# qc-tum/TNC

Measured on NVIDIA H100. Metric: pairwise contractions/sec (effective ZGEMM TFLOP/s in zgemm_tflops), higher is better.
Workload: dtype f64

## Files before the change

### tnc_b200/csrc/crt.cu

```cuda
#include "internal.h"
#include "sm90.h"
#include <cuda.h>
#include <algorithm>
#include <cmath>
#include <cstdio>
#include <cstdlib>

namespace tncb {

constexpr int CRT_MAX_MOD = 20;
static const int kModuli[CRT_MAX_MOD] = {256, 253, 251, 249, 247, 245, 241, 239, 233, 229,
                                         227, 223, 211, 199, 197, 193, 191, 181, 179, 173};
constexpr int CRT_BT = 128;
constexpr int CRT_BKB = 128;
template <bool KARA> struct CrtRing {
  static constexpr int STAGES = KARA ? 3 : 2;
};
constexpr int CRT_STG_ROW = 2 * CRT_BT + 16;
constexpr int CRT_STG_BYTES = 64 * CRT_STG_ROW;
constexpr int CRT_KCHUNK_MAX = 32768;
constexpr int CRT_G = 34;

struct CrtTables {
  int nmod;
  int a_bits_a, a_bits_b;
  int mod[CRT_MAX_MOD];
  int magic[CRT_MAX_MOD];
  double inv_mod[CRT_MAX_MOD];
  double rho1[CRT_MAX_MOD];
  double rho2[CRT_MAX_MOD];
  double p_scaled;
};

double crt_log2_product(int n) {
  double s = 0;
  for (int i = 0; i < n; i++) s += std::log2((double)kModuli[i]);
  return s;
}

void crt_choose(long long K, int want_bits, int nmod_force, int* nmod, int* bits_a, int* bits_b) {
  const double lk = std::log2((double)std::max<long long>(K, 1));
  auto needed = [&](int bits) {
    int q = 2;
    while (q < CRT_MAX_MOD && crt_log2_product(q) - 1e-9 < 2.0 * bits + lk + 3.0) q++;
    return q;
  };
  int n = nmod_force > 0 ? std::min(nmod_force, needed(53)) : needed(want_bits);
  n = std::max(2, std::min(n, CRT_MAX_MOD));
  int tot = (int)std::floor(crt_log2_product(n) - lk - 3.0 - 1e-9);
  tot = std::max(tot, 2);
  int a = std::min(want_bits, tot / 2), b = std::min(want_bits, tot - a);
  *nmod = n; *bits_a = a; *bits_b = b;
// ... 202 lines not shown
struct CrtGemmArgs {
  int8_t* R;
  int Np, Mp;
  int tiles_n, tiles_m, tile_m;
  int nmod, nkc, kb_per_chunk, num_kb;
  int total_items;
  int group;
  int negmod[CRT_MAX_MOD];
  int magic[CRT_MAX_MOD];
};

struct CrtItem { int mod_i, prod, kc, n0, m0; };
template <bool KARA>
__device__ __forceinline__ CrtItem crt_decode(const CrtGemmArgs& p, int item) {
  const int tiles = p.tiles_n * p.tiles_m;
  const int mk = item / tiles, t = item - mk * tiles;
  CrtItem it;
  const int mp = mk / p.nkc;
  it.kc = mk - mp * p.nkc;
  it.mod_i = KARA ? mp / 3 : mp; it.prod = KARA ? mp - it.mod_i * 3 : 0;
  const int per_band = p.group * p.tiles_m;
  const int band = t / per_band, first = band * p.group;
  const int gsize = min(p.group, p.tiles_n - first);
  const int r = t - band * per_band;
  it.n0 = (first + r % gsize) * CRT_BT;
  it.m0 = (r / gsize) * p.tile_m;
  return it;
}

template <bool KARA>
__global__ void __launch_bounds__(WG_THREADS, 1)
crt_gemm_kernel(const __grid_constant__ CUtensorMap mapB, const __grid_constant__ CUtensorMap mapA,
                const __grid_constant__ CrtGemmArgs p) {
  constexpr int STAGES = CrtRing<KARA>::STAGES;
  extern __shared__ __align__(1024) uint8_t crt_smem_raw[];
  uint8_t* smem = reinterpret_cast<uint8_t*>((reinterpret_cast<uintptr_t>(crt_smem_raw) + 1023) & ~(uintptr_t)1023);
  __shared__ uint64_t full_bar[STAGES], empty_bar[STAGES];
  const int wg = threadIdx.x >> 7, tid = threadIdx.x & 127;

  if (threadIdx.x == 0) {
    for (int s = 0; s < STAGES; s++) { wg_mbar_init(&full_bar[s], 1); wg_mbar_init(&empty_bar[s], 2); }
    asm volatile("fence.mbarrier_init.release.cluster;" ::: "memory");
  }
  __syncthreads();

  if (wg == 0) {
    wg_setmaxnreg_producer();
    if (tid != 0) return;
    int it = 0;
    for (int item = blockIdx.x; item < p.total_items; item += gridDim.x) {
      const CrtItem w = crt_decode<KARA>(p, item);
      const int kb0 = w.kc * p.kb_per_chunk, kb1 = min(p.num_kb, kb0 + p.kb_per_chunk);
      const int rowB = (KARA ? w.mod_i * 3 + w.prod : w.mod_i * 2) * p.Np + w.n0;
      const int rowA = (KARA ? w.mod_i * 3 + w.prod : w.mod_i * 3) * p.Mp + w.m0;
      for (int kb = kb0; kb < kb1; kb++, it++) {
        uint8_t* st = wg_produce_begin<STAGES, KARA>(smem, full_bar, empty_bar, it);
        uint64_t* bar = &full_bar[it % STAGES];
        const int kx = kb * CRT_BKB;
        uint8_t* a = st + WgStage<KARA>::A;
        wg_tma_2d(&mapB, bar, st, kx, rowB);
        if (KARA) {
          wg_tma_2d(&mapA, bar, a, kx, rowA);
          wg_tma_2d(&mapA, bar, a + WG_TILE, kx, rowA + WG_ROWS);
        } else {
          wg_tma_2d(&mapB, bar, st + WgStage<KARA>::B1, kx, rowB + p.Np);
          wg_tma_2d(&mapA, bar, a, kx, rowA);
          wg_tma_2d(&mapA, bar, a + WG_TILE, kx, rowA + p.Mp);
          wg_tma_2d(&mapA, bar, a + 2 * WG_TILE, kx, rowA + 2 * p.Mp);
        }
      }
    }
  } else {
    wg_setmaxnreg_consumer();
    const int c = wg - 1, wq = tid >> 5, lane = tid & 31;
    WgRing<STAGES, KARA> ring{smem, full_bar, empty_bar};
    uint8_t* stg = smem + STAGES * WgStage<KARA>::BYTES + c * CRT_STG_BYTES;
    uint32_t acc[128];
#pragma unroll
    for (int i = 0; i < 128; i++) acc[i] = 0u;
    for (int item = blockIdx.x; item < p.total_items; item += gridDim.x) {
      const CrtItem w = crt_decode<KARA>(p, item);
      const int kb0 = w.kc * p.kb_per_chunk, kb1 = min(p.num_kb, kb0 + p.kb_per_chunk);
      bool first = true;
      for (int kb = kb0; kb < kb1; kb++) ring.mma_stage(acc, c, first, tid == 0);
      ring.drain(tid == 0);
      const int negm = p.negmod[w.mod_i], magic = p.magic[w.mod_i];
      wg_bar_sync(1 + c);
#pragma unroll
      for (int j = 0; j < 32; j++) {
#pragma unroll
        for (int h = 0; h < 2; h++) {
          uint32_t b = 0;
#pragma unroll
          for (int e = 0; e < 2; e++) {
            const int a = (int)acc[4 * j + 2 * h + e];
            int t = __mulhi(a, magic) * negm + a;
            if (t > 127) t += negm;
            b |= ((uint32_t)t & 0xffu) << (8 * e);
          }
          const int r = wq * 16 + (lane >> 2) + 8 * h, col = 8 * j + 2 * (lane & 3);
          *reinterpret_cast<uint16_t*>(stg + r * CRT_STG_ROW + col) = (uint16_t)(b ^ 0x8080u);
        }
      }
      wg_bar_sync(1 + c);
      const long long nrow0 = (long long)w.n0 + c * 64;
#pragma unroll
      for (int i = 0; i < 8; i++) {
        const int q = i * 128 + tid, row = q >> 4, c16 = q & 15;
        int8_t* dst = KARA ? p.R + ((long long)((w.mod_i * p.nkc + w.kc) * 3 + w.prod) * p.Np + nrow0 + row) * p.Mp + w.m0 + c16 * 16
                           : p.R + ((long long)((w.mod_i * p.nkc + w.kc) * 2 + (c16 >> 3)) * p.Np + nrow0 + row) * p.Mp + w.m0 + (c16 & 7) * 16;
        *reinterpret_cast<uint4*>(dst) = *reinterpret_cast<const uint4*>(stg + row * CRT_STG_ROW + c16 * 16);
      }
    }
  }
}

struct CrtReconArgs {
  const int8_t* R;
  double2* C;
  const unsigned long long* max_n;
  const unsigned long long* max_m;
  long long rows, cols, ldc;
  long long Np, Mp;
  int nkc;
};

template <bool ONE_CHUNK, bool KARA>
__global__ void __launch_bounds__(256, 4)
crt_reconstruct_kernel(const __grid_constant__ CrtReconArgs a, const __grid_constant__ CrtTables T) {
  const long long cols4 = a.Mp >> 2;
  const long long idx = (long long)blockIdx.x * blockDim.x + threadIdx.x;
  const long long n = idx / cols4, m4 = (idx - n * cols4) * 4;
  if (n >= a.rows || m4 >= a.cols) return;
  double s1r[4], s2r[4], s1i[4], s2i[4];
#pragma unroll
  for (int j = 0; j < 4; j++) { s1r[j] = s2r[j] = s1i[j] = s2i[j] = 0.0; }
  const long long plane = a.Np * a.Mp;
  const int8_t* base = a.R + n * a.Mp + m4;
  const double bias = 4503599627370496.0 + (KARA ? 256.0 : 128.0) * (double)a.nkc;
  const double bias_i = 4503599627370496.0 + (KARA ? 384.0 : 128.0) * (double)a.nkc;
#pragma unroll 8
  for (int i = 0; i < T.nmod; i++) {
    uint32_t ur[4], ui[4];
    if (KARA) {
// ... 40 lines not shown
  double2* dst = a.C + n * a.ldc + m4;
  const double RMAGIC = 6755399441055744.0;
#pragma unroll
  for (int j = 0; j < 4; j++) {
    if (m4 + j >= a.cols) break;
    const int em = crt_exp_from_bits(a.max_m[m4 + j]);
    double2 out;
    if (en == kExpNonFinite || em == kExpNonFinite) {
      out = make_double2(__longlong_as_double(0x7ff8000000000000LL), __longlong_as_double(0x7ff8000000000000LL));
    } else {
      const double qr = ((s1r[j] + s2r[j]) + RMAGIC) - RMAGIC;
      const double qi = ((s1i[j] + s2i[j]) + RMAGIC) - RMAGIC;
      const double fr = (s1r[j] - qr) + s2r[j], fi = (s1i[j] - qi) + s2i[j];
      out = make_double2(scalbn(fr * T.p_scaled, en + em), scalbn(fi * T.p_scaled, en + em));
    }
    dst[j] = out;
  }
}

typedef CUresult (*EncodeTiledFn)(CUtensorMap*, CUtensorMapDataType, cuuint32_t, void*, const cuuint64_t*, const cuuint64_t*,
                                  const cuuint32_t*, const cuuint32_t*, CUtensorMapInterleave, CUtensorMapSwizzle,
                                  CUtensorMapL2promotion, CUtensorMapFloatOOBfill);
static EncodeTiledFn get_encode() {
  static EncodeTiledFn fn = nullptr;
  static bool tried = false;
  if (!tried) {
    tried = true;
    cudaDriverEntryPointQueryResult q;
    void* p = nullptr;
    if (cudaGetDriverEntryPoint("cuTensorMapEncodeTiled", &p, cudaEnableDefault, &q) == cudaSuccess) fn = (EncodeTiledFn)p;
  }
  return fn;
}
int wg_make_map(CUtensorMap* m, void* ptr, uint64_t rows, uint64_t kbytes) {
  EncodeTiledFn enc = get_encode();
  if (!enc) return fail(TNCB_ERR_CUDA, "cuTensorMapEncodeTiled is not available");
  cuuint64_t dims[2] = {kbytes, rows};
  cuuint64_t strides[1] = {kbytes};
  cuuint32_t box[2] = {(cuuint32_t)WG_BKB, (cuuint32_t)WG_ROWS};
  cuuint32_t estr[2] = {1, 1};
  CUresult r = enc(m, CU_TENSOR_MAP_DATA_TYPE_UINT8, 2, ptr, dims, strides, box, estr, CU_TENSOR_MAP_INTERLEAVE_NONE,
                   CU_TENSOR_MAP_SWIZZLE_128B, CU_TENSOR_MAP_L2_PROMOTION_L2_256B, CU_TENSOR_MAP_FLOAT_OOB_FILL_NONE);
  if (r != CUDA_SUCCESS) return fail(TNCB_ERR_CUDA, "cuTensorMapEncodeTiled failed: " + std::to_string((int)r));
  return TNCB_OK;
}

static inline long long round_up_ll(long long x, long long a) { return (x + a - 1) / a * a; }


int launch_k1_crt(tncb_ctx* ctx, const PairPlan& P, const double2* A, const double2* B, double2* C,
                  const long long* offAm, const long long* offBn, const long long* offAk, const long long* offBk) {
  int nmod, bits_a, bits_b;
  const int want = ctx->crt_tol > 0.0 ? crt_bits_for_tolerance(P.K, ctx->crt_tol) : ctx->crt_bits;
  crt_choose(P.K, want, ctx->crt_nmod_force, &nmod, &bits_a, &bits_b);
  CrtTables T;
  crt_make_tables(nmod, bits_a, bits_b, T);
  cudaStream_t st = ctx->stream;
  const long long Kp = round_up_ll(P.K, CRT_BKB);
  const int num_kb = (int)(Kp / CRT_BKB);
  const int ctas_max = std::max(1, ctx->sm_count);
  const bool kara = ctx->crt_products == 3 || (ctx->crt_products == 0 && Kp >= ctx->crt_kara_min_k);
  const int TM = kara ? 2 * CRT_BT : CRT_BT;
  const int NPB = kara ? 3 : 2, NPR = kara ? 3 : 2;
  const long long tiles_total = round_up_ll(P.N, CRT_BT) / CRT_BT * (round_up_ll(P.M, TM) / TM);
  int nkc = (int)((Kp + CRT_KCHUNK_MAX - 1) / CRT_KCHUNK_MAX);
  {
    const long long items = tiles_total * nmod * (kara ? 3 : 1);
    const long long want = ctas_max;
    if (items * nkc < want) nkc = (int)std::min<long long>((want + items - 1) / items, std::max(1, num_kb / 8));
    nkc = std::max(1, std::min(nkc, 32));
  }
  int kb_per_chunk = (num_kb + nkc - 1) / nkc;
  nkc = (num_kb + kb_per_chunk - 1) / kb_per_chunk;
  if ((long long)kb_per_chunk * CRT_BKB > CRT_KCHUNK_MAX) return fail(TNCB_ERR_UNSUPPORTED, "K too long for the int8 engine");

  const size_t budget = ctx->crt_ws_bytes;
  long long pn = round_up_ll(P.N, CRT_BT), pm = round_up_ll(P.M, TM);
  auto ws_bytes = [&](long long n_, long long m_) {
    return (size_t)nmod * (size_t)Kp * (size_t)(NPB * n_ + 3 * m_) + (size_t)nmod * nkc * NPR * (size_t)n_ * (size_t)m_;
  };
  while (ws_bytes(pn, pm) > budget && (pm > TM || pn > CRT_BT)) {
    if (pm >= pn && pm > TM) pm = round_up_ll(pm / 2, TM);
    else if (pn > CRT_BT) pn = round_up_ll(pn / 2, CRT_BT);
    else pm = round_up_ll(pm / 2, TM);
  }
  const size_t bytesB = (size_t)nmod * NPB * pn * Kp, bytesA = (size_t)nmod * 3 * pm * Kp;
  const size_t bytesR = (size_t)nmod * nkc * NPR * pn * pm;
  const size_t bytesE = (size_t)(pn + pm) * sizeof(unsigned long long);
  void *pb = nullptr, *pa = nullptr, *pr = nullptr, *pe = nullptr;
  int rc;
  if ((rc = ctx->arena.alloc(bytesB, &pb))) return rc;
  if ((rc = ctx->arena.alloc(bytesA, &pa))) { ctx->arena.free(pb, bytesB); return rc; }
  if ((rc = ctx->arena.alloc(bytesR, &pr))) { ctx->arena.free(pb, bytesB); ctx->arena.free(pa, bytesA); return rc; }
  if ((rc = ctx->arena.alloc(bytesE, &pe))) { ctx->arena.free(pb, bytesB); ctx->arena.free(pa, bytesA); ctx->arena.free(pr, bytesR); return rc; }
  auto cleanup = [&]() { ctx->arena.free(pb, bytesB); ctx->arena.free(pa, bytesA); ctx->arena.free(pr, bytesR); ctx->arena.free(pe, bytesE); };
  unsigned long long* max_n = (unsigned long long*)pe;
  unsigned long long* max_m = max_n + pn;

  static bool attr_done_dev[64] = {false};
  bool& attr_done = attr_done_dev[ctx->device & 63];
  const int smem_gemm4 = CrtRing<false>::STAGES * WgStage<false>::BYTES + 2 * CRT_STG_BYTES + 1024;
  const int smem_gemm3 = CrtRing<true>::STAGES * WgStage<true>::BYTES + 2 * CRT_STG_BYTES + 1024;
  const int smem_res = RES_ROWS * RES_RS * (int)sizeof(double2);
  if (!attr_done) {
    cudaError_t e = cudaFuncSetAttribute(crt_gemm_kernel<false>, cudaFuncAttributeMaxDynamicSharedMemorySize, smem_gemm4);
    if (e == cudaSuccess) e = cudaFuncSetAttribute(crt_gemm_kernel<true>, cudaFuncAttributeMaxDynamicSharedMemorySize, smem_gemm3);
    if (e == cudaSuccess) e = cudaFuncSetAttribute(crt_residue_kernel<2, false>, cudaFuncAttributeMaxDynamicSharedMemorySize, smem_res);
    if (e == cudaSuccess) e = cudaFuncSetAttribute(crt_residue_kernel<3, false>, cudaFuncAttributeMaxDynamicSharedMemorySize, smem_res);
    if (e == cudaSuccess) e = cudaFuncSetAttribute(crt_residue_kernel<2, true>, cudaFuncAttributeMaxDynamicSharedMemorySize, smem_res);
    if (e == cudaSuccess) e = cudaFuncSetAttribute(crt_residue_kernel<3, true>, cudaFuncAttributeMaxDynamicSharedMemorySize, smem_res);
    if (e != cudaSuccess) { cleanup(); return fail(TNCB_ERR_CUDA, cudaGetErrorString(e)); }
    attr_done = true;
  }
  auto lane_split = [](const LegList& kl, bool k_is_b, const LegList& fl) {
    auto p2 = [](long long d) { int b = 0; while ((2LL << b) <= d && b < 5) b++; return b; };
    const long long ks = kl.n ? (k_is_b ? kl.sb[kl.n - 1] : kl.sa[kl.n - 1]) : (1LL << 62);
    const long long fs = fl.n ? fl.sa[fl.n - 1] : (1LL << 62);
    if (ks <= fs) return kl.n ? p2(kl.dim[kl.n - 1]) : 0;
    return 0;
  };
  const int lk_b = lane_split(P.k, true, P.n), lk_a = lane_split(P.k, false, P.m);
  ctx->last_int8_ops = 0.0; ctx->last_nmod = nmod; ctx->last_products = kara ? 3 : 4;
  bool timed = false;

  for (long long n0 = 0; n0 < P.N; n0 += pn) {
    const long long nrows = std::min(pn, P.N - n0);
    const long long Np = round_up_ll(nrows, CRT_BT);
    if (Np != nrows) cudaMemsetAsync(pb, 0, (size_t)nmod * NPB * Np * Kp, st);
    cudaMemsetAsync(max_n, 0, (size_t)nrows * sizeof(unsigned long long), st);
    {
      dim3 g((unsigned)((nrows + RES_ROWS - 1) / RES_ROWS), (unsigned)(Kp / RES_K));
      crt_rowmax_kernel<<<g, 256, 0, st>>>(B, offBn + n0, offBk, nrows, P.K, lk_b, max_n);
      if (kara) crt_residue_kernel<2, true><<<g, 256, smem_res, st>>>(B, offBn + n0, offBk, nrows, P.K, Np, Kp, max_n, bits_b, lk_b, T, (int8_t*)pb);
      else crt_residue_kernel<2, false><<<g, 256, smem_res, st>>>(B, offBn + n0, offBk, nrows, P.K, Np, Kp, max_n, bits_b, lk_b, T, (int8_t*)pb);
    }
    ctx->launches += 2;
    CUtensorMap mapB;
    if ((rc = wg_make_map(&mapB, pb, (uint64_t)nmod * NPB * Np, (uint64_t)Kp))) { cleanup(); return rc; }
    for (long long m0 = 0; m0 < P.M; m0 += pm) {
      const long long mcols = std::min(pm, P.M - m0);
      const long long Mp = round_up_ll(mcols, TM);
      if (Mp != mcols) cudaMemsetAsync(pa, 0, (size_t)nmod * 3 * Mp * Kp, st);
      cudaMemsetAsync(max_m, 0, (size_t)mcols * sizeof(unsigned long long), st);
      {
        dim3 g((unsigned)((mcols + RES_ROWS - 1) / RES_ROWS), (unsigned)(Kp / RES_K));
        crt_rowmax_kernel<<<g, 256, 0, st>>>(A, offAm + m0, offAk, mcols, P.K, lk_a, max_m);
        if (kara) crt_residue_kernel<3, true><<<g, 256, smem_res, st>>>(A, offAm + m0, offAk, mcols, P.K, Mp, Kp, max_m, bits_a, lk_a, T, (int8_t*)pa);
        else crt_residue_kernel<3, false><<<g, 256, smem_res, st>>>(A, offAm + m0, offAk, mcols, P.K, Mp, Kp, max_m, bits_a, lk_a, T, (int8_t*)pa);
      }
      ctx->launches += 2;
      CUtensorMap mapA;
      if ((rc = wg_make_map(&mapA, pa, (uint64_t)nmod * 3 * Mp, (uint64_t)Kp))) { cleanup(); return rc; }
      CrtGemmArgs g;
      g.R = (int8_t*)pr; g.Np = (int)Np; g.Mp = (int)Mp;
      g.tiles_n = (int)(Np / CRT_BT); g.tiles_m = (int)(Mp / TM); g.tile_m = TM;
      g.nmod = nmod; g.nkc = nkc; g.kb_per_chunk = kb_per_chunk; g.num_kb = num_kb;
      const long long items = (long long)g.tiles_n * g.tiles_m * nmod * nkc * (kara ? 3 : 1);
      if (items > 0x7fffffffLL) { cleanup(); return fail(TNCB_ERR_UNSUPPORTED, "too many work items"); }
      g.total_items = (int)items;
      g.group = ctx->crt_group;
      for (int i = 0; i < CRT_MAX_MOD; i++) { g.negmod[i] = -T.mod[i]; g.magic[i] = T.magic[i]; }
      const unsigned grid = (unsigned)std::min<long long>(ctas_max, items);
      const double ops = 2.0 * (kara ? 3.0 : 4.0) * (double)nmod * (double)Np * (double)Mp * (double)Kp;
      const bool time_this = ctx->time_gemm == 2 || (ctx->time_gemm == 1 && !timed);
      if (time_this) gemm_timer_begin(ctx);
      if (kara) crt_gemm_kernel<true><<<grid, WG_THREADS, smem_gemm3, st>>>(mapB, mapA, g);
      else crt_gemm_kernel<false><<<grid, WG_THREADS, smem_gemm4, st>>>(mapB, mapA, g);
      cudaError_t e = cudaGetLastError();
      if (time_this) { gemm_timer_end(ctx, ops); timed = true; }
      if (e != cudaSuccess) { cleanup(); return fail(TNCB_ERR_CUDA, std::string("crt_gemm_kernel launch: ") + cudaGetErrorString(e)); }
      ctx->last_int8_ops += ops;
      CrtReconArgs r;
      r.R = (const int8_t*)pr; r.C = C + n0 * P.M + m0; r.max_n = max_n; r.max_m = max_m;
      r.rows = nrows; r.cols = mcols; r.ldc = P.M; r.Np = Np; r.Mp = Mp; r.nkc = nkc;
      const long long threads = nrows * (Mp / 4);
      const unsigned rg = (unsigned)((threads + 255) / 256);
      if (kara) {
        if (nkc == 1) crt_reconstruct_kernel<true, true><<<rg, 256, 0, st>>>(r, T);
        else crt_reconstruct_kernel<false, true><<<rg, 256, 0, st>>>(r, T);
      } else {
        if (nkc == 1) crt_reconstruct_kernel<true, false><<<rg, 256, 0, st>>>(r, T);
        else crt_reconstruct_kernel<false, false><<<rg, 256, 0, st>>>(r, T);
      }
      ctx->launches += 2;
    }
// ... 10 lines not shown
```

### tnc_b200/csrc/ozaki.cu

```cuda
#include "internal.h"
#include "sm90.h"
#include <cuda.h>
#include <algorithm>
#include <cstdio>
#include <cstdlib>

namespace tncb {

constexpr int OZ_BT = 128;
constexpr int OZ_BKB = 128;
constexpr int OZ_STAGES = 2;
constexpr int OZ_KCHUNK = 8192;
constexpr int OZ_MAX_S = 8;
constexpr int kOzExpMin = -1000;

__global__ void oz_rowexp_kernel(const double2* __restrict__ src, const long long* __restrict__ off_row,
                                 const long long* __restrict__ off_k, long long rows, long long K, int* __restrict__ exps) {
  const long long row = (long long)blockIdx.x * (blockDim.x >> 5) + (threadIdx.x >> 5);
  const int lane = threadIdx.x & 31;
  if (row >= rows) return;
  const long long base = off_row[row];
  double m = 0.0;
  for (long long k = lane; k < K; k += 32) {
    const double2 v = __ldg(src + base + __ldg(off_k + k));
// ... 68 lines not shown
__global__ void __launch_bounds__(WG_THREADS, 1)
oz_gemm_kernel(const __grid_constant__ CUtensorMap mapB, const __grid_constant__ CUtensorMap mapA,
               const __grid_constant__ OzArgs p) {
  extern __shared__ __align__(1024) uint8_t oz_smem_raw[];
  uint8_t* smem = reinterpret_cast<uint8_t*>((reinterpret_cast<uintptr_t>(oz_smem_raw) + 1023) & ~(uintptr_t)1023);
  __shared__ uint64_t full_bar[OZ_STAGES], empty_bar[OZ_STAGES];
  __shared__ int col_exp[OZ_BT];
  const int wg = threadIdx.x >> 7, tid = threadIdx.x & 127;
  const int n0 = blockIdx.y * OZ_BT, m0 = blockIdx.x * OZ_BT;
  const int S = p.S;
  const int kb_per_chunk = OZ_KCHUNK / OZ_BKB;
  const int nkc = (p.num_kb + kb_per_chunk - 1) / kb_per_chunk;

  if (threadIdx.x == 0) {
    for (int s = 0; s < OZ_STAGES; s++) { wg_mbar_init(&full_bar[s], 1); wg_mbar_init(&empty_bar[s], 2); }
    asm volatile("fence.mbarrier_init.release.cluster;" ::: "memory");
  }
  if (threadIdx.x < OZ_BT) {
    const long long gm = (long long)m0 + threadIdx.x;
    col_exp[threadIdx.x] = gm < p.M ? p.exp_m[gm] : 0;
  }
  __syncthreads();

  if (wg == 0) {
    wg_setmaxnreg_producer();
    if (tid != 0) return;
    int it = 0;
    for (int t = 0; t < S; t++)
      for (int kc = 0; kc < nkc; kc++) {
        const int kb0 = kc * kb_per_chunk, kb1 = min(p.num_kb, kb0 + kb_per_chunk);
        for (int pp = 0; pp <= t; pp++) {
          const int qq = t - pp;
          for (int kb = kb0; kb < kb1; kb++, it++) {
            uint8_t* st = wg_produce_begin<OZ_STAGES, false>(smem, full_bar, empty_bar, it);
            uint64_t* bar = &full_bar[it % OZ_STAGES];
            uint8_t* a = st + WgStage<false>::A;
            const int kx = kb * OZ_BKB;
            wg_tma_2d(&mapB, bar, st, kx, (0 * S + pp) * p.Np + n0);
            wg_tma_2d(&mapB, bar, st + WgStage<false>::B1, kx, (1 * S + pp) * p.Np + n0);
            wg_tma_2d(&mapA, bar, a, kx, (0 * S + qq) * p.Mp + m0);
            wg_tma_2d(&mapA, bar, a + WG_TILE, kx, (1 * S + qq) * p.Mp + m0);
            wg_tma_2d(&mapA, bar, a + 2 * WG_TILE, kx, (2 * S + qq) * p.Mp + m0);
          }
        }
      }
  } else {
    wg_setmaxnreg_consumer();
    const int c = wg - 1, wq = tid >> 5, lane = tid & 31;
    WgRing<OZ_STAGES, false> ring{smem, full_bar, empty_bar};
    long long gn[2];
    bool row_ok[2];
    int en[2];
#pragma unroll
    for (int h = 0; h < 2; h++) {
      gn[h] = (long long)n0 + c * 64 + wq * 16 + (lane >> 2) + 8 * h;
      row_ok[h] = gn[h] < p.N;
      en[h] = row_ok[h] ? p.exp_n[gn[h]] : 0;
    }
    uint32_t acc[128];
#pragma unroll
    for (int i = 0; i < 128; i++) acc[i] = 0u;
    int f = 0;
    for (int t = 0; t < S; t++) {
      const int row_exp[2] = {en[0] - 7 * (t + 2), en[1] - 7 * (t + 2)};
      for (int kc = 0; kc < nkc; kc++, f++) {
        const int kb0 = kc * kb_per_chunk, kb1 = min(p.num_kb, kb0 + kb_per_chunk);
        bool first = true;
        for (int pp = 0; pp <= t; pp++)
          for (int kb = kb0; kb < kb1; kb++) ring.mma_stage(acc, c, first, tid == 0);
        ring.drain(tid == 0);
#pragma unroll
        for (int h = 0; h < 2; h++) {
          if (!row_ok[h]) continue;
          double2* crow = p.C + gn[h] * p.M + m0;
#pragma unroll
          for (int j = 0; j < 16; j++) {
#pragma unroll
            for (int e = 0; e < 2; e++) {
              const int col = 8 * j + 2 * (lane & 3) + e;
              if ((long long)m0 + col < p.M) {
                const int sc = row_exp[h] + col_exp[col];
                double2 v = make_double2(scalbn((double)(int)acc[4 * j + 2 * h + e], sc), scalbn((double)(int)acc[4 * (j + 16) + 2 * h + e], sc));
// ... 6 lines not shown
      }
    }
  }
}

int launch_k1_ozaki(tncb_ctx* ctx, const PairPlan& P, const double2* A, const double2* B, double2* C, int S,
                    const long long* offAm, const long long* offBn, const long long* offAk, const long long* offBk) {
  if (S < 2) S = 2;
  if (S > OZ_MAX_S) S = OZ_MAX_S;
  const long long Np = (P.N + OZ_BT - 1) / OZ_BT * OZ_BT, Mp = (P.M + OZ_BT - 1) / OZ_BT * OZ_BT;
  const long long Kp = (P.K + OZ_BKB - 1) / OZ_BKB * OZ_BKB;
  const size_t bytesB = (size_t)2 * S * Np * Kp, bytesA = (size_t)3 * S * Mp * Kp;
  const size_t bytesE = (size_t)(Np + Mp) * sizeof(int);
  void *pb = nullptr, *pa = nullptr, *pe = nullptr;
  int rc;
  if ((rc = ctx->arena.alloc(bytesB, &pb))) return rc;
  if ((rc = ctx->arena.alloc(bytesA, &pa))) { ctx->arena.free(pb, bytesB); return rc; }
  if ((rc = ctx->arena.alloc(bytesE, &pe))) { ctx->arena.free(pb, bytesB); ctx->arena.free(pa, bytesA); return rc; }
  auto cleanup = [&]() { ctx->arena.free(pb, bytesB); ctx->arena.free(pa, bytesA); ctx->arena.free(pe, bytesE); };
  int* exp_n = (int*)pe;
  int* exp_m = exp_n + Np;
  cudaStream_t st = ctx->stream;
  if (Np != P.N) cudaMemsetAsync(pb, 0, bytesB, st);
  if (Mp != P.M) cudaMemsetAsync(pa, 0, bytesA, st);
  oz_rowexp_kernel<<<(unsigned)((P.N + 7) / 8), 256, 0, st>>>(B, offBn, offBk, P.N, P.K, exp_n);
  oz_rowexp_kernel<<<(unsigned)((P.M + 7) / 8), 256, 0, st>>>(A, offAm, offAk, P.M, P.K, exp_m);
  {
    const unsigned gx = (unsigned)((Kp / 16 + 127) / 128);
    oz_slice_kernel<2><<<dim3((unsigned)P.N, gx), 128, 0, st>>>(B, offBn, offBk, P.N, P.K, Np, Kp, exp_n, S, (int8_t*)pb);
    oz_slice_kernel<3><<<dim3((unsigned)P.M, gx), 128, 0, st>>>(A, offAm, offAk, P.M, P.K, Mp, Kp, exp_m, S, (int8_t*)pa);
  }
  ctx->launches += 4;
  CUtensorMap mapB, mapA;
  if ((rc = wg_make_map(&mapB, pb, (uint64_t)2 * S * Np, (uint64_t)Kp)) || (rc = wg_make_map(&mapA, pa, (uint64_t)3 * S * Mp, (uint64_t)Kp))) { cleanup(); return rc; }
  OzArgs a;
  a.C = C; a.exp_n = exp_n; a.exp_m = exp_m; a.M = P.M; a.N = P.N; a.Np = (int)Np; a.Mp = (int)Mp;
  a.num_kb = (int)(Kp / OZ_BKB); a.S = S;
  const int smem_bytes = OZ_STAGES * WgStage<false>::BYTES + 1024;
  cudaError_t e = cudaFuncSetAttribute(oz_gemm_kernel, cudaFuncAttributeMaxDynamicSharedMemorySize, smem_bytes);
  if (e != cudaSuccess) { cleanup(); return fail(TNCB_ERR_CUDA, cudaGetErrorString(e)); }
  const double ops = 2.0 * 4.0 * (S * (S + 1) / 2) * (double)Np * (double)Mp * (double)Kp;
  if (ctx->time_gemm) gemm_timer_begin(ctx);
  oz_gemm_kernel<<<dim3((unsigned)(Mp / OZ_BT), (unsigned)(Np / OZ_BT)), WG_THREADS, smem_bytes, st>>>(mapB, mapA, a);
  if (ctx->time_gemm) gemm_timer_end(ctx, ops);
  ctx->last_int8_ops = ops; ctx->last_nmod = 0;
  ctx->launches++;
  e = cudaGetLastError();
  cleanup();
  if (e != cudaSuccess) return fail(TNCB_ERR_CUDA, std::string("oz_gemm_kernel: ") + cudaGetErrorString(e));
  return TNCB_OK;
}

}
```

### tnc_b200/csrc/sm90.h

```cpp
#pragma once
#include <cstdint>
#include <cuda.h>

namespace tncb {

constexpr int WG_ROWS = 128;
constexpr int WG_BKB = 128;
constexpr int WG_TILE = WG_ROWS * WG_BKB;
constexpr int WG_THREADS = 384;

template <bool KARA> struct WgStage {
  static constexpr int B1 = WG_TILE;
  static constexpr int A = KARA ? WG_TILE : 2 * WG_TILE;
  static constexpr int BYTES = KARA ? 3 * WG_TILE : 5 * WG_TILE;
};

__device__ __forceinline__ uint32_t wg_smem(const void* p) { return (uint32_t)__cvta_generic_to_shared(p); }
__device__ __forceinline__ void wg_mbar_init(uint64_t* bar, int count) {
  asm volatile("mbarrier.init.shared::cta.b64 [%0], %1;" ::"r"(wg_smem(bar)), "r"(count));
}
__device__ __forceinline__ void wg_mbar_expect_tx(uint64_t* bar, uint32_t bytes) {
  asm volatile("mbarrier.arrive.expect_tx.shared::cta.b64 _, [%0], %1;" ::"r"(wg_smem(bar)), "r"(bytes) : "memory");
}
__device__ __forceinline__ void wg_mbar_arrive(uint64_t* bar) {
  asm volatile("mbarrier.arrive.shared::cta.b64 _, [%0];" ::"r"(wg_smem(bar)) : "memory");
}
__device__ __forceinline__ void wg_mbar_wait(uint64_t* bar, uint32_t parity) {
  uint32_t done = 0;
  while (!done) {
    asm volatile(
        "{\n\t.reg .pred P1;\n\t"
        "mbarrier.try_wait.parity.shared::cta.b64 P1, [%1], %2;\n\t"
        "selp.u32 %0, 1, 0, P1;\n\t}"
        : "=r"(done) : "r"(wg_smem(bar)), "r"(parity) : "memory");
  }
}
__device__ __forceinline__ void wg_tma_2d(const CUtensorMap* map, uint64_t* bar, void* smem, int c0, int c1) {
  asm volatile("cp.async.bulk.tensor.2d.shared::cluster.global.mbarrier::complete_tx::bytes [%0], [%1, {%3, %4}], [%2];"
               ::"r"(wg_smem(smem)), "l"(map), "r"(wg_smem(bar)), "r"(c0), "r"(c1) : "memory");
}
__device__ __forceinline__ void wg_bar_sync(int id) { asm volatile("bar.sync %0, 128;" ::"r"(id) : "memory"); }

__device__ __forceinline__ uint64_t wg_desc(const void* smem) {
  uint64_t d = 0;
  d |= (uint64_t)((wg_smem(smem) & 0x3FFFF) >> 4);
  d |= (uint64_t)1 << 16;
  d |= (uint64_t)(1024 >> 4) << 32;
  d |= (uint64_t)1 << 62;
  return d;
}

__device__ __forceinline__ void wg_fence() { asm volatile("wgmma.fence.sync.aligned;" ::: "memory"); }
__device__ __forceinline__ void wg_commit() { asm volatile("wgmma.commit_group.sync.aligned;" ::: "memory"); }
template <int N> __device__ __forceinline__ void wg_wait() { asm volatile("wgmma.wait_group.sync.aligned %0;" ::"n"(N) : "memory"); }

__device__ __forceinline__ void wg_mma_s8_m64n256k32(uint32_t (&d)[128], uint64_t da, uint64_t db, uint32_t accumulate) {
  asm volatile(
      "{\n\t.reg .pred p;\n\tsetp.ne.b32 p, %130, 0;\n\t"
      "wgmma.mma_async.sync.aligned.m64n256k32.s32.s8.s8 "
      "{"
      "%0,%1,%2,%3,%4,%5,%6,%7,%8,%9,%10,%11,%12,%13,%14,%15,"
      "%16,%17,%18,%19,%20,%21,%22,%23,%24,%25,%26,%27,%28,%29,%30,%31,"
      "%32,%33,%34,%35,%36,%37,%38,%39,%40,%41,%42,%43,%44,%45,%46,%47,"
      "%48,%49,%50,%51,%52,%53,%54,%55,%56,%57,%58,%59,%60,%61,%62,%63,"
      "%64,%65,%66,%67,%68,%69,%70,%71,%72,%73,%74,%75,%76,%77,%78,%79,"
      "%80,%81,%82,%83,%84,%85,%86,%87,%88,%89,%90,%91,%92,%93,%94,%95,"
      "%96,%97,%98,%99,%100,%101,%102,%103,%104,%105,%106,%107,%108,%109,%110,%111,"
      "%112,%113,%114,%115,%116,%117,%118,%119,%120,%121,%122,%123,%124,%125,%126,%127"
      "}, %128, %129, p;\n\t}"
      : "+r"(d[0]), "+r"(d[1]), "+r"(d[2]), "+r"(d[3]), "+r"(d[4]), "+r"(d[5]), "+r"(d[6]), "+r"(d[7]),
        "+r"(d[8]), "+r"(d[9]), "+r"(d[10]), "+r"(d[11]), "+r"(d[12]), "+r"(d[13]), "+r"(d[14]), "+r"(d[15]),
        "+r"(d[16]), "+r"(d[17]), "+r"(d[18]), "+r"(d[19]), "+r"(d[20]), "+r"(d[21]), "+r"(d[22]), "+r"(d[23]),
        "+r"(d[24]), "+r"(d[25]), "+r"(d[26]), "+r"(d[27]), "+r"(d[28]), "+r"(d[29]), "+r"(d[30]), "+r"(d[31]),
        "+r"(d[32]), "+r"(d[33]), "+r"(d[34]), "+r"(d[35]), "+r"(d[36]), "+r"(d[37]), "+r"(d[38]), "+r"(d[39]),
        "+r"(d[40]), "+r"(d[41]), "+r"(d[42]), "+r"(d[43]), "+r"(d[44]), "+r"(d[45]), "+r"(d[46]), "+r"(d[47]),
        "+r"(d[48]), "+r"(d[49]), "+r"(d[50]), "+r"(d[51]), "+r"(d[52]), "+r"(d[53]), "+r"(d[54]), "+r"(d[55]),
        "+r"(d[56]), "+r"(d[57]), "+r"(d[58]), "+r"(d[59]), "+r"(d[60]), "+r"(d[61]), "+r"(d[62]), "+r"(d[63]),
        "+r"(d[64]), "+r"(d[65]), "+r"(d[66]), "+r"(d[67]), "+r"(d[68]), "+r"(d[69]), "+r"(d[70]), "+r"(d[71]),
        "+r"(d[72]), "+r"(d[73]), "+r"(d[74]), "+r"(d[75]), "+r"(d[76]), "+r"(d[77]), "+r"(d[78]), "+r"(d[79]),
        "+r"(d[80]), "+r"(d[81]), "+r"(d[82]), "+r"(d[83]), "+r"(d[84]), "+r"(d[85]), "+r"(d[86]), "+r"(d[87]),
        "+r"(d[88]), "+r"(d[89]), "+r"(d[90]), "+r"(d[91]), "+r"(d[92]), "+r"(d[93]), "+r"(d[94]), "+r"(d[95]),
        "+r"(d[96]), "+r"(d[97]), "+r"(d[98]), "+r"(d[99]), "+r"(d[100]), "+r"(d[101]), "+r"(d[102]), "+r"(d[103]),
        "+r"(d[104]), "+r"(d[105]), "+r"(d[106]), "+r"(d[107]), "+r"(d[108]), "+r"(d[109]), "+r"(d[110]), "+r"(d[111]),
        "+r"(d[112]), "+r"(d[113]), "+r"(d[114]), "+r"(d[115]), "+r"(d[116]), "+r"(d[117]), "+r"(d[118]), "+r"(d[119]),
        "+r"(d[120]), "+r"(d[121]), "+r"(d[122]), "+r"(d[123]), "+r"(d[124]), "+r"(d[125]), "+r"(d[126]), "+r"(d[127])
      : "l"(da), "l"(db), "r"(accumulate));
}

template <int STAGES, bool KARA>
struct WgRing {
  uint8_t* smem; uint64_t* full; uint64_t* empty;
  int it = 0, pending = -1;

  __device__ __forceinline__ void mma_stage(uint32_t (&acc)[128], int wg, bool& first, bool signal) {
    const int s = it % STAGES;
    wg_mbar_wait(&full[s], (it / STAGES) & 1);
    const uint8_t* st = smem + s * WgStage<KARA>::BYTES;
    const uint8_t* b0 = st + wg * 64 * WG_BKB;
    const uint8_t* a = st + WgStage<KARA>::A;
    wg_fence();
    if (KARA) {
      const uint64_t d_b = wg_desc(b0), d_a = wg_desc(a);
#pragma unroll
      for (int k = 0; k < WG_BKB / 32; k++) {
        wg_mma_s8_m64n256k32(acc, d_b + (uint64_t)(k * 2), d_a + (uint64_t)(k * 2), first ? 0u : 1u);
        first = false;
      }
    } else {
      const uint64_t d_br = wg_desc(b0), d_bi = wg_desc(b0 + WgStage<KARA>::B1);
      const uint64_t d_x = wg_desc(a + WG_TILE), d_y = wg_desc(a);
#pragma unroll
      for (int k = 0; k < WG_BKB / 32; k++) {
        const uint64_t ko = (uint64_t)(k * 2);
        wg_mma_s8_m64n256k32(acc, d_br + ko, d_x + ko, first ? 0u : 1u);
        first = false;
        wg_mma_s8_m64n256k32(acc, d_bi + ko, d_y + ko, 1u);
      }
    }
    wg_commit();
    wg_wait<1>();
    if (pending >= 0 && signal) wg_mbar_arrive(&empty[pending]);
    pending = s;
    it++;
  }
  __device__ __forceinline__ void drain(bool signal) {
    wg_wait<0>();
    if (pending >= 0 && signal) wg_mbar_arrive(&empty[pending]);
    pending = -1;
  }
};

template <int STAGES, bool KARA>
__device__ __forceinline__ uint8_t* wg_produce_begin(uint8_t* smem, uint64_t* full, uint64_t* empty, int it) {
  const int s = it % STAGES;
  if (it >= STAGES) wg_mbar_wait(&empty[s], ((it / STAGES) - 1) & 1);
  wg_mbar_expect_tx(&full[s], WgStage<KARA>::BYTES);
  return smem + s * WgStage<KARA>::BYTES;
}

__device__ __forceinline__ void wg_setmaxnreg_producer() { asm volatile("setmaxnreg.dec.sync.aligned.u32 40;"); }
__device__ __forceinline__ void wg_setmaxnreg_consumer() { asm volatile("setmaxnreg.inc.sync.aligned.u32 232;"); }

int wg_make_map(CUtensorMap* m, void* ptr, uint64_t rows, uint64_t kbytes);

}
```

Before: 5596.

## Deepen CRT 4-product ring with 64-byte K stages and shuffle-based epilogue

The non-Karatsuba CRT GEMM now uses five pipeline stages of 64 K-bytes each, with SWIZZLE_64B tensor maps and descriptors, in place of two stages of 128. The freed shared memory comes partly from removing the staging buffer. The epilogue now packs residues in registers, transposes them across quad lanes with warp shuffles, and writes 16-byte stores straight to global memory, dropping the shared-memory staging and its named barriers. The aim is better latency hiding in the TMA/WGMMA pipeline and a cheaper epilogue, at the cost of more barrier round-trips per K and more shuffle work.

Result: faster. 5829, median of 6 (+4.2%).

```diff
diff --git a/tnc_b200/csrc/crt.cu b/tnc_b200/csrc/crt.cu
--- a/tnc_b200/csrc/crt.cu
+++ b/tnc_b200/csrc/crt.cu
@@ -12,12 +12,26 @@
 static const int kModuli[CRT_MAX_MOD] = {256, 253, 251, 249, 247, 245, 241, 239, 233, 229,
                                          227, 223, 211, 199, 197, 193, 191, 181, 179, 173};
 constexpr int CRT_BT = 128;
-constexpr int CRT_BKB = 128;
+constexpr int CRT_BKB = WG_BKB;
+#ifndef CRT_RING3_STAGES
+#define CRT_RING3_STAGES 3
+#endif
+#ifndef CRT_RING3_BK
+#define CRT_RING3_BK 128
+#endif
+#ifndef CRT_RING4_STAGES
+#define CRT_RING4_STAGES 5
+#endif
+#ifndef CRT_RING4_BK
+#define CRT_RING4_BK 64
+#endif
 template <bool KARA> struct CrtRing {
-  static constexpr int STAGES = KARA ? 3 : 2;
+  static constexpr int STAGES = KARA ? CRT_RING3_STAGES : CRT_RING4_STAGES;
+  static constexpr int BK = KARA ? CRT_RING3_BK : CRT_RING4_BK;
+  using Stage = WgStage<KARA, BK>;
+  static constexpr int SMEM = STAGES * Stage::BYTES + 1024;
+  static_assert(SMEM <= 232448 - 1024, "stage ring exceeds the per-block shared memory of sm_90");
 };
-constexpr int CRT_STG_ROW = 2 * CRT_BT + 16;
-constexpr int CRT_STG_BYTES = 64 * CRT_STG_ROW;
 constexpr int CRT_KCHUNK_MAX = 32768;
 constexpr int CRT_G = 34;
 
@@ -286,7 +300,8 @@
 __global__ void __launch_bounds__(WG_THREADS, 1)
 crt_gemm_kernel(const __grid_constant__ CUtensorMap mapB, const __grid_constant__ CUtensorMap mapA,
                 const __grid_constant__ CrtGemmArgs p) {
-  constexpr int STAGES = CrtRing<KARA>::STAGES;
+  constexpr int STAGES = CrtRing<KARA>::STAGES, BK = CrtRing<KARA>::BK, SUB = CRT_BKB / BK;
+  using Stage = typename CrtRing<KARA>::Stage;
   extern __shared__ __align__(1024) uint8_t crt_smem_raw[];
   uint8_t* smem = reinterpret_cast<uint8_t*>((reinterpret_cast<uintptr_t>(crt_smem_raw) + 1023) & ~(uintptr_t)1023);
   __shared__ uint64_t full_bar[STAGES], empty_bar[STAGES];
@@ -307,28 +322,29 @@
       const int kb0 = w.kc * p.kb_per_chunk, kb1 = min(p.num_kb, kb0 + p.kb_per_chunk);
       const int rowB = (KARA ? w.mod_i * 3 + w.prod : w.mod_i * 2) * p.Np + w.n0;
       const int rowA = (KARA ? w.mod_i * 3 + w.prod : w.mod_i * 3) * p.Mp + w.m0;
-      for (int kb = kb0; kb < kb1; kb++, it++) {
-        uint8_t* st = wg_produce_begin<STAGES, KARA>(smem, full_bar, empty_bar, it);
+      for (int ks = kb0 * SUB; ks < kb1 * SUB; ks++, it++) {
+        uint8_t* st = wg_produce_begin<STAGES, KARA, BK>(smem, full_bar, empty_bar, it);
         uint64_t* bar = &full_bar[it % STAGES];
-        const int kx = kb * CRT_BKB;
-        uint8_t* a = st + WgStage<KARA>::A;
+        const int kx = ks * BK;
+        uint8_t* a = st + Stage::A;
         wg_tma_2d(&mapB, bar, st, kx, rowB);
         if (KARA) {
           wg_tma_2d(&mapA, bar, a, kx, rowA);
-          wg_tma_2d(&mapA, bar, a + WG_TILE, kx, rowA + WG_ROWS);
+          wg_tma_2d(&mapA, bar, a + Stage::TILE, kx, rowA + WG_ROWS);
         } else {
-          wg_tma_2d(&mapB, bar, st + WgStage<KARA>::B1, kx, rowB + p.Np);
+          wg_tma_2d(&mapB, bar, st + Stage::B1, kx, rowB + p.Np);
           wg_tma_2d(&mapA, bar, a, kx, rowA);
-          wg_tma_2d(&mapA, bar, a + WG_TILE, kx, rowA + p.Mp);
-          wg_tma_2d(&mapA, bar, a + 2 * WG_TILE, kx, rowA + 2 * p.Mp);
+          wg_tma_2d(&mapA, bar, a + Stage::TILE, kx, rowA + p.Mp);
+          wg_tma_2d(&mapA, bar, a + 2 * Stage::TILE, kx, rowA + 2 * p.Mp);
         }
       }
     }
   } else {
     wg_setmaxnreg_consumer();
     const int c = wg - 1, wq = tid >> 5, lane = tid & 31;
-    WgRing<STAGES, KARA> ring{smem, full_bar, empty_bar};
-    uint8_t* stg = smem + STAGES * WgStage<KARA>::BYTES + c * CRT_STG_BYTES;
+    const int q = lane & 3;
+    const bool q0 = q & 1, q1 = q & 2;
+    WgRing<STAGES, KARA, BK> ring{smem, full_bar, empty_bar};
     uint32_t acc[128];
 #pragma unroll
     for (int i = 0; i < 128; i++) acc[i] = 0u;
@@ -336,34 +352,51 @@
       const CrtItem w = crt_decode<KARA>(p, item);
       const int kb0 = w.kc * p.kb_per_chunk, kb1 = min(p.num_kb, kb0 + p.kb_per_chunk);
       bool first = true;
-      for (int kb = kb0; kb < kb1; kb++) ring.mma_stage(acc, c, first, tid == 0);
+      for (int ks = kb0 * SUB; ks < kb1 * SUB; ks++) ring.mma_stage(acc, c, first, tid == 0);
       ring.drain(tid == 0);
       const int negm = p.negmod[w.mod_i], magic = p.magic[w.mod_i];
-      wg_bar_sync(1 + c);
-#pragma unroll
-      for (int j = 0; j < 32; j++) {
+      int8_t* row_base[2];
+#pragma unroll
+      for (int h = 0; h < 2; h++) {
+        const long long n = (long long)w.n0 + c * 64 + wq * 16 + (lane >> 2) + 8 * h;
+        row_base[h] = KARA ? p.R + ((long long)((w.mod_i * p.nkc + w.kc) * 3 + w.prod) * p.Np + n) * p.Mp + w.m0
+                           : p.R + ((long long)((w.mod_i * p.nkc + w.kc) * 2) * p.Np + n) * p.Mp + w.m0;
+      }
+#pragma unroll
+      for (int i = 0; i < 4; i++) {
 #pragma unroll
         for (int h = 0; h < 2; h++) {
-          uint32_t b = 0;
-#pragma unroll
-          for (int e = 0; e < 2; e++) {
-            const int a = (int)acc[4 * j + 2 * h + e];
-            int t = __mulhi(a, magic) * negm + a;
-            if (t > 127) t += negm;
-            b |= ((uint32_t)t & 0xffu) << (8 * e);
+          uint32_t x[4];
+#pragma unroll
+          for (int k = 0; k < 4; k++) {
+            uint32_t u = 0;
+#pragma unroll
+            for (int jj = 0; jj < 2; jj++) {
+#pragma unroll
+              for (int e = 0; e < 2; e++) {
+                const int a = (int)acc[4 * (8 * i + 2 * k + jj) + 2 * h + e];
+                int t = __mulhi(a, magic) * negm + a;
+                if (t > 127) t += negm;
+                u |= (((uint32_t)t & 0xffu) ^ 0x80u) << (8 * (2 * jj + e));
+              }
+            }
+            x[k] = u;
           }
-          const int r = wq * 16 + (lane >> 2) + 8 * h, col = 8 * j + 2 * (lane & 3);
-          *reinterpret_cast<uint16_t*>(stg + r * CRT_STG_ROW + col) = (uint16_t)(b ^ 0x8080u);
+          const uint32_t r0 = __shfl_xor_sync(0xffffffffu, q0 ? x[0] : x[1], 1);
+          const uint32_t r1 = __shfl_xor_sync(0xffffffffu, q0 ? x[2] : x[3], 1);
+          const uint32_t a0 = q0 ? r0 : x[0], a1 = q0 ? x[1] : r0;
+          const uint32_t b0 = q0 ? r1 : x[2], b1 = q0 ? x[3] : r1;
+          const uint32_t g0 = __shfl_xor_sync(0xffffffffu, q1 ? a0 : b0, 2);
+          const uint32_t g1 = __shfl_xor_sync(0xffffffffu, q1 ? a1 : b1, 2);
+          const uint32_t k0 = q1 ? b0 : a0, k1 = q1 ? b1 : a1;
+          const uint32_t y0 = q1 ? g0 : k0, y1 = q1 ? g1 : k1, y2 = q1 ? k0 : g0, y3 = q1 ? k1 : g1;
+          const uint4 v = make_uint4(__byte_perm(y0, y1, 0x5410), __byte_perm(y2, y3, 0x5410),
+                                     __byte_perm(y0, y1, 0x7632), __byte_perm(y2, y3, 0x7632));
+          const int cc = 4 * i + q;
+          int8_t* dst = KARA ? row_base[h] + cc * 16
+                             : row_base[h] + (i >= 2 ? (long long)p.Np * p.Mp : 0LL) + (cc & 7) * 16;
+          *reinterpret_cast<uint4*>(dst) = v;
         }
-      }
-      wg_bar_sync(1 + c);
-      const long long nrow0 = (long long)w.n0 + c * 64;
-#pragma unroll
-      for (int i = 0; i < 8; i++) {
-        const int q = i * 128 + tid, row = q >> 4, c16 = q & 15;
-        int8_t* dst = KARA ? p.R + ((long long)((w.mod_i * p.nkc + w.kc) * 3 + w.prod) * p.Np + nrow0 + row) * p.Mp + w.m0 + c16 * 16
-                           : p.R + ((long long)((w.mod_i * p.nkc + w.kc) * 2 + (c16 >> 3)) * p.Np + nrow0 + row) * p.Mp + w.m0 + (c16 & 7) * 16;
-        *reinterpret_cast<uint4*>(dst) = *reinterpret_cast<const uint4*>(stg + row * CRT_STG_ROW + c16 * 16);
       }
     }
   }
@@ -470,18 +503,23 @@
   }
   return fn;
 }
+template <int BK>
 int wg_make_map(CUtensorMap* m, void* ptr, uint64_t rows, uint64_t kbytes) {
+  static_assert(BK == 128 || BK == 64, "SWIZZLE_128B or SWIZZLE_64B");
   EncodeTiledFn enc = get_encode();
   if (!enc) return fail(TNCB_ERR_CUDA, "cuTensorMapEncodeTiled is not available");
   cuuint64_t dims[2] = {kbytes, rows};
   cuuint64_t strides[1] = {kbytes};
-  cuuint32_t box[2] = {(cuuint32_t)WG_BKB, (cuuint32_t)WG_ROWS};
+  cuuint32_t box[2] = {(cuuint32_t)BK, (cuuint32_t)WG_ROWS};
   cuuint32_t estr[2] = {1, 1};
   CUresult r = enc(m, CU_TENSOR_MAP_DATA_TYPE_UINT8, 2, ptr, dims, strides, box, estr, CU_TENSOR_MAP_INTERLEAVE_NONE,
-                   CU_TENSOR_MAP_SWIZZLE_128B, CU_TENSOR_MAP_L2_PROMOTION_L2_256B, CU_TENSOR_MAP_FLOAT_OOB_FILL_NONE);
+                   BK == 128 ? CU_TENSOR_MAP_SWIZZLE_128B : CU_TENSOR_MAP_SWIZZLE_64B, CU_TENSOR_MAP_L2_PROMOTION_L2_256B,
+                   CU_TENSOR_MAP_FLOAT_OOB_FILL_NONE);
   if (r != CUDA_SUCCESS) return fail(TNCB_ERR_CUDA, "cuTensorMapEncodeTiled failed: " + std::to_string((int)r));
   return TNCB_OK;
 }
+template int wg_make_map<128>(CUtensorMap*, void*, uint64_t, uint64_t);
+template int wg_make_map<64>(CUtensorMap*, void*, uint64_t, uint64_t);
 
 static inline long long round_up_ll(long long x, long long a) { return (x + a - 1) / a * a; }
 
@@ -537,8 +575,7 @@
 
   static bool attr_done_dev[64] = {false};
   bool& attr_done = attr_done_dev[ctx->device & 63];
-  const int smem_gemm4 = CrtRing<false>::STAGES * WgStage<false>::BYTES + 2 * CRT_STG_BYTES + 1024;
-  const int smem_gemm3 = CrtRing<true>::STAGES * WgStage<true>::BYTES + 2 * CRT_STG_BYTES + 1024;
+  const int smem_gemm4 = CrtRing<false>::SMEM, smem_gemm3 = CrtRing<true>::SMEM;
   const int smem_res = RES_ROWS * RES_RS * (int)sizeof(double2);
   if (!attr_done) {
     cudaError_t e = cudaFuncSetAttribute(crt_gemm_kernel<false>, cudaFuncAttributeMaxDynamicSharedMemorySize, smem_gemm4);
@@ -574,7 +611,8 @@
     }
     ctx->launches += 2;
     CUtensorMap mapB;
-    if ((rc = wg_make_map(&mapB, pb, (uint64_t)nmod * NPB * Np, (uint64_t)Kp))) { cleanup(); return rc; }
+    if ((rc = kara ? wg_make_map<CrtRing<true>::BK>(&mapB, pb, (uint64_t)nmod * NPB * Np, (uint64_t)Kp)
+                   : wg_make_map<CrtRing<false>::BK>(&mapB, pb, (uint64_t)nmod * NPB * Np, (uint64_t)Kp))) { cleanup(); return rc; }
     for (long long m0 = 0; m0 < P.M; m0 += pm) {
       const long long mcols = std::min(pm, P.M - m0);
       const long long Mp = round_up_ll(mcols, TM);
@@ -588,7 +626,8 @@
       }
       ctx->launches += 2;
       CUtensorMap mapA;
-      if ((rc = wg_make_map(&mapA, pa, (uint64_t)nmod * 3 * Mp, (uint64_t)Kp))) { cleanup(); return rc; }
+      if ((rc = kara ? wg_make_map<CrtRing<true>::BK>(&mapA, pa, (uint64_t)nmod * 3 * Mp, (uint64_t)Kp)
+                     : wg_make_map<CrtRing<false>::BK>(&mapA, pa, (uint64_t)nmod * 3 * Mp, (uint64_t)Kp))) { cleanup(); return rc; }
       CrtGemmArgs g;
       g.R = (int8_t*)pr; g.Np = (int)Np; g.Mp = (int)Mp;
       g.tiles_n = (int)(Np / CRT_BT); g.tiles_m = (int)(Mp / TM); g.tile_m = TM;
diff --git a/tnc_b200/csrc/ozaki.cu b/tnc_b200/csrc/ozaki.cu
--- a/tnc_b200/csrc/ozaki.cu
+++ b/tnc_b200/csrc/ozaki.cu
@@ -124,22 +124,23 @@
         for (int pp = 0; pp <= t; pp++) {
           const int qq = t - pp;
           for (int kb = kb0; kb < kb1; kb++, it++) {
-            uint8_t* st = wg_produce_begin<OZ_STAGES, false>(smem, full_bar, empty_bar, it);
+            using Stage = WgStage<false, OZ_BKB>;
+            uint8_t* st = wg_produce_begin<OZ_STAGES, false, OZ_BKB>(smem, full_bar, empty_bar, it);
             uint64_t* bar = &full_bar[it % OZ_STAGES];
-            uint8_t* a = st + WgStage<false>::A;
+            uint8_t* a = st + Stage::A;
             const int kx = kb * OZ_BKB;
             wg_tma_2d(&mapB, bar, st, kx, (0 * S + pp) * p.Np + n0);
-            wg_tma_2d(&mapB, bar, st + WgStage<false>::B1, kx, (1 * S + pp) * p.Np + n0);
+            wg_tma_2d(&mapB, bar, st + Stage::B1, kx, (1 * S + pp) * p.Np + n0);
             wg_tma_2d(&mapA, bar, a, kx, (0 * S + qq) * p.Mp + m0);
-            wg_tma_2d(&mapA, bar, a + WG_TILE, kx, (1 * S + qq) * p.Mp + m0);
-            wg_tma_2d(&mapA, bar, a + 2 * WG_TILE, kx, (2 * S + qq) * p.Mp + m0);
+            wg_tma_2d(&mapA, bar, a + Stage::TILE, kx, (1 * S + qq) * p.Mp + m0);
+            wg_tma_2d(&mapA, bar, a + 2 * Stage::TILE, kx, (2 * S + qq) * p.Mp + m0);
           }
         }
       }
   } else {
     wg_setmaxnreg_consumer();
     const int c = wg - 1, wq = tid >> 5, lane = tid & 31;
-    WgRing<OZ_STAGES, false> ring{smem, full_bar, empty_bar};
+    WgRing<OZ_STAGES, false, OZ_BKB> ring{smem, full_bar, empty_bar};
     long long gn[2];
     bool row_ok[2];
     int en[2];
@@ -212,11 +213,11 @@
   }
   ctx->launches += 4;
   CUtensorMap mapB, mapA;
-  if ((rc = wg_make_map(&mapB, pb, (uint64_t)2 * S * Np, (uint64_t)Kp)) || (rc = wg_make_map(&mapA, pa, (uint64_t)3 * S * Mp, (uint64_t)Kp))) { cleanup(); return rc; }
+  if ((rc = wg_make_map<OZ_BKB>(&mapB, pb, (uint64_t)2 * S * Np, (uint64_t)Kp)) || (rc = wg_make_map<OZ_BKB>(&mapA, pa, (uint64_t)3 * S * Mp, (uint64_t)Kp))) { cleanup(); return rc; }
   OzArgs a;
   a.C = C; a.exp_n = exp_n; a.exp_m = exp_m; a.M = P.M; a.N = P.N; a.Np = (int)Np; a.Mp = (int)Mp;
   a.num_kb = (int)(Kp / OZ_BKB); a.S = S;
-  const int smem_bytes = OZ_STAGES * WgStage<false>::BYTES + 1024;
+  const int smem_bytes = OZ_STAGES * WgStage<false, OZ_BKB>::BYTES + 1024;
   cudaError_t e = cudaFuncSetAttribute(oz_gemm_kernel, cudaFuncAttributeMaxDynamicSharedMemorySize, smem_bytes);
   if (e != cudaSuccess) { cleanup(); return fail(TNCB_ERR_CUDA, cudaGetErrorString(e)); }
   const double ops = 2.0 * 4.0 * (S * (S + 1) / 2) * (double)Np * (double)Mp * (double)Kp;
diff --git a/tnc_b200/csrc/sm90.h b/tnc_b200/csrc/sm90.h
--- a/tnc_b200/csrc/sm90.h
+++ b/tnc_b200/csrc/sm90.h
@@ -6,13 +6,14 @@
 
 constexpr int WG_ROWS = 128;
 constexpr int WG_BKB = 128;
-constexpr int WG_TILE = WG_ROWS * WG_BKB;
 constexpr int WG_THREADS = 384;
 
-template <bool KARA> struct WgStage {
-  static constexpr int B1 = WG_TILE;
-  static constexpr int A = KARA ? WG_TILE : 2 * WG_TILE;
-  static constexpr int BYTES = KARA ? 3 * WG_TILE : 5 * WG_TILE;
+template <bool KARA, int BK> struct WgStage {
+  static_assert(BK == 128 || BK == 64, "a stage is 128 (SWIZZLE_128B) or 64 (SWIZZLE_64B) K bytes deep");
+  static constexpr int TILE = WG_ROWS * BK;
+  static constexpr int B1 = TILE;
+  static constexpr int A = KARA ? TILE : 2 * TILE;
+  static constexpr int BYTES = KARA ? 3 * TILE : 5 * TILE;
 };
 
 __device__ __forceinline__ uint32_t wg_smem(const void* p) { return (uint32_t)__cvta_generic_to_shared(p); }
@@ -39,14 +40,15 @@
   asm volatile("cp.async.bulk.tensor.2d.shared::cluster.global.mbarrier::complete_tx::bytes [%0], [%1, {%3, %4}], [%2];"
                ::"r"(wg_smem(smem)), "l"(map), "r"(wg_smem(bar)), "r"(c0), "r"(c1) : "memory");
 }
-__device__ __forceinline__ void wg_bar_sync(int id) { asm volatile("bar.sync %0, 128;" ::"r"(id) : "memory"); }
 
+template <int BK>
 __device__ __forceinline__ uint64_t wg_desc(const void* smem) {
+  static_assert(BK == 128 || BK == 64, "SWIZZLE_128B or SWIZZLE_64B");
   uint64_t d = 0;
   d |= (uint64_t)((wg_smem(smem) & 0x3FFFF) >> 4);
   d |= (uint64_t)1 << 16;
-  d |= (uint64_t)(1024 >> 4) << 32;
-  d |= (uint64_t)1 << 62;
+  d |= (uint64_t)((8 * BK) >> 4) << 32;
+  d |= (uint64_t)(BK == 128 ? 1 : 2) << 62;
   return d;
 }
 
@@ -87,30 +89,31 @@
       : "l"(da), "l"(db), "r"(accumulate));
 }
 
-template <int STAGES, bool KARA>
+template <int STAGES, bool KARA, int BK>
 struct WgRing {
+  using Stage = WgStage<KARA, BK>;
   uint8_t* smem; uint64_t* full; uint64_t* empty;
   int it = 0, pending = -1;
 
   __device__ __forceinline__ void mma_stage(uint32_t (&acc)[128], int wg, bool& first, bool signal) {
     const int s = it % STAGES;
     wg_mbar_wait(&full[s], (it / STAGES) & 1);
-    const uint8_t* st = smem + s * WgStage<KARA>::BYTES;
-    const uint8_t* b0 = st + wg * 64 * WG_BKB;
-    const uint8_t* a = st + WgStage<KARA>::A;
+    const uint8_t* st = smem + s * Stage::BYTES;
+    const uint8_t* b0 = st + wg * 64 * BK;
+    const uint8_t* a = st + Stage::A;
     wg_fence();
     if (KARA) {
-      const uint64_t d_b = wg_desc(b0), d_a = wg_desc(a);
+      const uint64_t d_b = wg_desc<BK>(b0), d_a = wg_desc<BK>(a);
 #pragma unroll
-      for (int k = 0; k < WG_BKB / 32; k++) {
+      for (int k = 0; k < BK / 32; k++) {
         wg_mma_s8_m64n256k32(acc, d_b + (uint64_t)(k * 2), d_a + (uint64_t)(k * 2), first ? 0u : 1u);
         first = false;
       }
     } else {
-      const uint64_t d_br = wg_desc(b0), d_bi = wg_desc(b0 + WgStage<KARA>::B1);
-      const uint64_t d_x = wg_desc(a + WG_TILE), d_y = wg_desc(a);
+      const uint64_t d_br = wg_desc<BK>(b0), d_bi = wg_desc<BK>(b0 + Stage::B1);
+      const uint64_t d_x = wg_desc<BK>(a + Stage::TILE), d_y = wg_desc<BK>(a);
 #pragma unroll
-      for (int k = 0; k < WG_BKB / 32; k++) {
+      for (int k = 0; k < BK / 32; k++) {
         const uint64_t ko = (uint64_t)(k * 2);
         wg_mma_s8_m64n256k32(acc, d_br + ko, d_x + ko, first ? 0u : 1u);
         first = false;
@@ -130,17 +133,17 @@
   }
 };
 
-template <int STAGES, bool KARA>
+template <int STAGES, bool KARA, int BK>
 __device__ __forceinline__ uint8_t* wg_produce_begin(uint8_t* smem, uint64_t* full, uint64_t* empty, int it) {
   const int s = it % STAGES;
   if (it >= STAGES) wg_mbar_wait(&empty[s], ((it / STAGES) - 1) & 1);
-  wg_mbar_expect_tx(&full[s], WgStage<KARA>::BYTES);
-  return smem + s * WgStage<KARA>::BYTES;
+  wg_mbar_expect_tx(&full[s], WgStage<KARA, BK>::BYTES);
+  return smem + s * WgStage<KARA, BK>::BYTES;
 }
 
 __device__ __forceinline__ void wg_setmaxnreg_producer() { asm volatile("setmaxnreg.dec.sync.aligned.u32 40;"); }
 __device__ __forceinline__ void wg_setmaxnreg_consumer() { asm volatile("setmaxnreg.inc.sync.aligned.u32 232;"); }
 
-int wg_make_map(CUtensorMap* m, void* ptr, uint64_t rows, uint64_t kbytes);
+template <int BK> int wg_make_map(CUtensorMap* m, void* ptr, uint64_t rows, uint64_t kbytes);
 
 }
```
